# labhamlet/wavjepa

Measured on AMD Instinct MI355X. Metric: jepa_pretrain_clips_per_sec, higher is better.
Workload: dtype bf16; 1 GPU; WavJEPA-base JEPA pre-training step, 2.01 s @16 kHz white-noise clips (32159 samples -> 200 tokens), 256 clips per GPU (32 sources x 8 crops), AudioSet masker, random-init weights; workload_name=2s-bf16, global_batch=256, seq_len=200, parallelism=dp1, persistent_gemm_workgroups_per_xcd=32

## Files before the change

### wavjepa_amd/csrc/conv0.hip

```cpp
#include <string.h>
#include "conv_pieces.h"
#include "../../include/wavjepa_hip.h"

namespace {

constexpr int TC = 256;
constexpr int NTH = 256;

struct Geo {
    int N, C_in, L, C, k, stride, L_out, P;
    long clip_stride;
};

template <int NT, class T>
__device__ __forceinline__ void stage_steps(T* xs, const bf16_t* __restrict__ audio, const Geo& g, int n, int t0, int span) {
    stage_chunk<NT>(xs, audio, (long)n * g.clip_stride, g.C_in, g.L, (long)t0 * g.stride, span);
}

__host__ __device__ constexpr long fwd_record(int C, int taps, int want_yx) { return want_yx ? 2L * C + (long)C * taps + taps : 2L * C; }

constexpr int STATS_SLOTS = 768;
inline int stats_tcs(int N, int L_out, int C_in) {
    static int forced = -1;
    if (forced < 0) forced = wj_lab_env_int("WJ_CONV0_STATS_TCS", 0);
    if (forced >= 32) return forced / 32 * 32;
    int chunks = (STATS_SLOTS + N / 2) / (N > 0 ? N : 1);
    const int most = (L_out + 255) / 256;
    chunks = chunks < 1 ? 1 : (chunks > most ? most : chunks);
    const int tcs = ((L_out + chunks - 1) / chunks + 31) / 32 * 32;
    const int cap = 2176 / (C_in > 0 ? C_in : 1) / 32 * 32;
    return tcs > cap ? (cap < 32 ? 32 : cap) : tcs;
}
inline int stats_chunks(int L_out, int TCS) { return (L_out + TCS - 1) / TCS; }
template <int TAPS>
__global__ __launch_bounds__(256) void conv0_gram_kernel(const bf16_t* __restrict__ audio, double* __restrict__ part, Geo g, int span, int TCS) {
    extern __shared__ __attribute__((aligned(16))) bf16_t xa[];
    constexpr int G = TAPS + TAPS * TAPS;
    __shared__ double red[4][G];
    const int n = blockIdx.y, t0 = blockIdx.x * TCS;
    stage_steps<256>(xa, audio, g, n, t0, span);
    __syncthreads();
    const int lane = threadIdx.x & 63, wave = threadIdx.x >> 6;
    const int tcount = min(TCS, g.L_out - t0);
    for (int p = lane; p < G; p += 64) {
        const bool one = p < TAPS;
        const int qa = one ? p : (p - TAPS) / TAPS, qb = one ? 0 : (p - TAPS) - qa * TAPS;
        const int offa = tap_at(qa, g.k, span), offb = tap_at(qb, g.k, span);
        double acc = 0.0;
        for (int t = wave; t < tcount; t += 4) {
            const float a = bf2f(xa[offa + t * g.stride]);
            const float b = one ? 1.0f : bf2f(xa[offb + t * g.stride]);
            acc += (double)(a * b);
        }
        red[wave][p] = acc;
    }
    __syncthreads();
    double* o = part + ((long)n * gridDim.x + blockIdx.x) * G;
    for (int p = threadIdx.x; p < G; p += 256) o[p] = (red[0][p] + red[1][p]) + (red[2][p] + red[3][p]);
}

template <int TAPS>
__global__ __launch_bounds__(256) void conv0_stats_from_gram_kernel(const double* __restrict__ gram, const bf16_t* __restrict__ wsrc,
                                                                    float* __restrict__ sums, float* __restrict__ yx, float* __restrict__ x1,
                                                                    Geo g) {
    constexpr int G = TAPS + TAPS * TAPS;
    __shared__ double gs[G];
    const int n = blockIdx.y;
    for (int p = threadIdx.x; p < G; p += 256) gs[p] = gram[(long)n * G + p];
    __syncthreads();
    if (x1 && blockIdx.x == 0 && threadIdx.x < TAPS) x1[(long)n * TAPS + threadIdx.x] = (float)gs[threadIdx.x];
    const int c = blockIdx.x * 256 + threadIdx.x;
    if (c >= g.C) return;
    double w[TAPS];
#pragma unroll
    for (int q = 0; q < TAPS; ++q) w[q] = (double)bf2f(wsrc[(long)c * TAPS + q]);
    double s1 = 0.0, s2 = 0.0;
#pragma unroll
    for (int q = 0; q < TAPS; ++q) s1 += w[q] * gs[q];
#pragma unroll
    for (int q = 0; q < TAPS; ++q) {
        double v = 0.0;
#pragma unroll
        for (int k = 0; k < TAPS; ++k) v += w[k] * gs[TAPS + k * TAPS + q];
        s2 += v * w[q];
        if (yx) yx[((long)n * g.C + c) * TAPS + q] = (float)v;
    }
    sums[((long)n * g.C + c) * 2] = (float)s1;
    sums[((long)n * g.C + c) * 2 + 1] = (float)fmax(s2, 0.0);
}

template <int TAPS>
__global__ __launch_bounds__(256) void conv0_stats_mfma_kernel(const bf16_t* __restrict__ audio, const bf16_t* __restrict__ wsrc,
                                                               float* __restrict__ part, int want_yx, Geo g, int span, int TCS) {
    extern __shared__ __attribute__((aligned(16))) bf16_t xa[];
    constexpr int QT = (TAPS + 15) / 16;
    const int n = blockIdx.y, t0 = blockIdx.x * TCS;
    const long rec = fwd_record(g.C, TAPS, want_yx);
    float* sums = part + ((long)n * gridDim.x + blockIdx.x) * rec;
    float* yx = want_yx ? sums + 2L * g.C : nullptr;
    float* x1 = want_yx ? yx + (long)g.C * TAPS : nullptr;
    stage_steps<256>(xa, audio, g, n, t0, span);
    __syncthreads();
    const int lane = threadIdx.x & 63, wave = threadIdx.x >> 6, i = lane & 15, gq = lane >> 4;
    const int tcount = min(TCS, g.L_out - t0);
    const bf16_t zero = f2bf(0.f);
    int offc[8];
    bool okc[8];
    tap_map<TAPS>(offc, okc, 8 * gq, 1, g.k, span);
    int offq[QT];
    bool okq[QT];
    tap_map<TAPS>(offq, okq, i, 16, g.k, span);
    const int ntile = g.C / 16;
    for (int ctg = wave * 8; ctg < ntile; ctg += 32) {
        bf16x8 wf[8];
#pragma unroll
        for (int u = 0; u < 8; ++u)
#pragma unroll
            for (int j = 0; j < 8; ++j)
                wf[u][j] = (ctg + u < ntile && okc[j]) ? wsrc[(long)((ctg + u) * 16 + i) * TAPS + 8 * gq + j] : zero;
        f32x4 yxa[8][QT];
        float s1[8], s2[8], xs1[QT];
#pragma unroll
        for (int u = 0; u < 8; ++u) {
            s1[u] = s2[u] = 0.f;
#pragma unroll
            for (int qt = 0; qt < QT; ++qt) yxa[u][qt] = f32x4{0.f, 0.f, 0.f, 0.f};
        }
#pragma unroll
        for (int qt = 0; qt < QT; ++qt) xs1[qt] = 0.f;
        for (int tb = 0; tb < tcount; tb += 32) {
            bf16x8 p0, p1, pq[QT];
            const bool v0 = tb + i < tcount, v1 = tb + 16 + i < tcount;
#pragma unroll
            for (int j = 0; j < 8; ++j) {
                p0[j] = (v0 && okc[j]) ? xa[offc[j] + (tb + i) * g.stride] : zero;
                p1[j] = (v1 && okc[j]) ? xa[offc[j] + (tb + 16 + i) * g.stride] : zero;
            }
#pragma unroll
            for (int qt = 0; qt < QT; ++qt)
#pragma unroll
                for (int j = 0; j < 8; ++j) {
                    const int tt = tb + (j < 4 ? 4 * gq + j : 12 + 4 * gq + j);
                    pq[qt][j] = (okq[qt] && tt < tcount) ? xa[offq[qt] + tt * g.stride] : zero;
                }
            if (yx && ctg == 0) {
#pragma unroll
                for (int qt = 0; qt < QT; ++qt)
#pragma unroll
                    for (int j = 0; j < 8; ++j) xs1[qt] += bf2f(pq[qt][j]);
            }
#pragma unroll
            for (int u = 0; u < 8; ++u) {
                const f32x4 z4 = f32x4{0.f, 0.f, 0.f, 0.f};
                const f32x4 d0 = __builtin_amdgcn_mfma_f32_16x16x32_bf16(p0, wf[u], z4, 0, 0, 0);
                const f32x4 d1 = __builtin_amdgcn_mfma_f32_16x16x32_bf16(p1, wf[u], z4, 0, 0, 0);
                bf16x8 yq;
#pragma unroll
                for (int r = 0; r < 4; ++r) {
                    yq[r] = f2bf(d0[r]);
                    yq[4 + r] = f2bf(d1[r]);
                    const float a = bf2f(yq[r]), b = bf2f(yq[4 + r]);
                    s1[u] += a + b;
                    s2[u] = fmaf(a, a, fmaf(b, b, s2[u]));
                }
                if (yx) {
#pragma unroll
                    for (int qt = 0; qt < QT; ++qt) yxa[u][qt] = __builtin_amdgcn_mfma_f32_16x16x32_bf16(pq[qt], yq, yxa[u][qt], 0, 0, 0);
                }
            }
        }
#pragma unroll
        for (int u = 0; u < 8; ++u) {
            if (ctg + u >= ntile) continue;
            const int c = (ctg + u) * 16 + i;
            float a = s1[u], b = s2[u];
            a += __shfl_xor(a, 16, 64); a += __shfl_xor(a, 32, 64);
            b += __shfl_xor(b, 16, 64); b += __shfl_xor(b, 32, 64);
            if (gq == 0) {
                sums[c * 2 + 0] = a;
                sums[c * 2 + 1] = b;
            }
            if (yx) {
#pragma unroll
                for (int qt = 0; qt < QT; ++qt)
#pragma unroll
                    for (int r = 0; r < 4; ++r) {
                        const int q = 16 * qt + 4 * gq + r;
                        if (q < TAPS) yx[(long)c * TAPS + q] = yxa[u][qt][r];
                    }
            }
        }
        if (yx && ctg == 0) {
#pragma unroll
            for (int qt = 0; qt < QT; ++qt) {
                float v = xs1[qt];
                v += __shfl_xor(v, 16, 64); v += __shfl_xor(v, 32, 64);
                if (gq == 0 && okq[qt]) x1[16 * qt + i] = v;
            }
        }
    }
}

template <int TAPS>
__global__ __launch_bounds__(NTH) void conv0_apply_kernel(const bf16_t* __restrict__ audio, const bf16_t* __restrict__ wsrc,
                                                          const float* __restrict__ gamma, const float* __restrict__ beta,
                                                          const float* __restrict__ sums, bf16_t* __restrict__ act,
                                                          float* __restrict__ mean_o, float* __restrict__ rstd_o, Geo g,
                                                          int span_max, float eps) {
    extern __shared__ float xs[];
    const int n = blockIdx.y, t0 = blockIdx.x * TC;
    const int half = threadIdx.x >> 7, cl = threadIdx.x & 127;
    stage_steps<NTH>(xs, audio, g, n, t0, span_max);
    __syncthreads();
    const int tmax = min(TC, g.P - t0);
    const float invL = 1.0f / (float)g.L_out;
    for (int cb = 0; cb < g.C; cb += 512) {
        const int c4 = cb + cl * 4;
        if (c4 >= g.C) continue;
        float w[4][TAPS];
        load_weights(w, wsrc, c4);
        float mu[4], rs[4], ga[4], be[4];
// ... 126 lines not shown
    extern __shared__ float xs[];
    int* tl = reinterpret_cast<int*>(xs + BR * TAPS);
    float* red = xs + BR * TAPS + BR;
    const int n = blockIdx.y;
    const int first = rows ? row_off[n] : 0;
    const int cnt = rows ? row_off[n + 1] - first : g.L_out;
    const int j0 = blockIdx.x * BR;
    if (j0 >= cnt) return;
    const int jn = min(BR, cnt - j0);
    const int half = threadIdx.x >> 7, cl = threadIdx.x & 127;
    for (int j = threadIdx.x; j < jn; j += NTH) tl[j] = rows ? rows[first + j0 + j] - n * g.P : j0 + j;
    __syncthreads();
    for (int idx = threadIdx.x; idx < jn * TAPS; idx += NTH) {
        const int j = idx / TAPS;
        xs[idx] = bf2f(audio[(long)n * g.clip_stride + (long)tl[j] * g.stride + tap_at(idx - j * TAPS, g.k, g.L)]);
    }
    __syncthreads();
    for (int cb = 0; cb < g.C; cb += 512) {
        const int c4 = cb + cl * 4;
        const bool live = c4 < g.C;
        float acc[4][TAPS], a1[4] = {0, 0, 0, 0}, a2[4] = {0, 0, 0, 0};
#pragma unroll
        for (int j = 0; j < 4; ++j)
#pragma unroll
            for (int tp = 0; tp < TAPS; ++tp) acc[j][tp] = 0.f;
        if (live) {
            float w[4][TAPS];
            load_weights(w, wsrc, c4);
            float mu[4], rs[4], ga[4], be[4];
#pragma unroll
            for (int j = 0; j < 4; ++j) {
                mu[j] = mean[(long)n * g.C + c4 + j]; rs[j] = rstd[(long)n * g.C + c4 + j];
                ga[j] = gamma[c4 + j]; be[j] = beta[c4 + j];
            }
            constexpr int RB = 4;
            for (int jj0 = half; jj0 < jn; jj0 += 2 * RB) {
                bf16x4 dv[RB];
#pragma unroll
                for (int u = 0; u < RB; ++u) {
                    const int jq = jj0 + 2 * u < jn ? jj0 + 2 * u : jj0;
                    dv[u] = *reinterpret_cast<const bf16x4*>(dact + ((long)n * g.P + tl[jq]) * g.C + c4);
                }
#pragma unroll
                for (int u = 0; u < RB; ++u) {
                    const int jj = jj0 + 2 * u;
                    if (jj >= jn) break;
                    float x[TAPS], y[4];
#pragma unroll
                    for (int tp = 0; tp < TAPS; ++tp) x[tp] = xs[jj * TAPS + tp];
                    conv_row(y, x, [&](int j, int q) { return w[j][q]; }, nullptr);
                    const bf16x4 d = dv[u];
#pragma unroll
                    for (int j = 0; j < 4; ++j) {
                        const float xh = (y[j] - mu[j]) * rs[j];
                        const float dz = bf2f(d[j]) * gelu_grad_f(xh * ga[j] + be[j]);
                        a1[j] += dz;
                        a2[j] = fmaf(dz, xh, a2[j]);
#pragma unroll
                        for (int tp = 0; tp < TAPS; ++tp) acc[j][tp] = fmaf(dz, x[tp], acc[j][tp]);
                    }
                }
            }
        }
        __syncthreads();
        if (live && half == 1) {
#pragma unroll
            for (int j = 0; j < 4; ++j) {
                red[(j * (2 + TAPS) + 0) * 128 + cl] = a1[j];
                red[(j * (2 + TAPS) + 1) * 128 + cl] = a2[j];
#pragma unroll
                for (int tp = 0; tp < TAPS; ++tp) red[(j * (2 + TAPS) + 2 + tp) * 128 + cl] = acc[j][tp];
            }
        }
        __syncthreads();
        if (live && half == 0) {
#pragma unroll
            for (int j = 0; j < 4; ++j) {
                float* o = ws + (((long)n * gridDim.x + blockIdx.x) * g.C + c4 + j) * (2 + TAPS);
                o[0] = a1[j] + red[(j * (2 + TAPS) + 0) * 128 + cl];
                o[1] = a2[j] + red[(j * (2 + TAPS) + 1) * 128 + cl];
#pragma unroll
                for (int tp = 0; tp < TAPS; ++tp) o[2 + tp] = acc[j][tp] + red[(j * (2 + TAPS) + 2 + tp) * 128 + cl];
            }
        }
    }
}

template <int TAPS>
__global__ __launch_bounds__(256) void conv0_bwd_final_kernel(const float* __restrict__ gamma, const float* __restrict__ mean,
                                                              const float* __restrict__ rstd, const float* __restrict__ ws,
                                                              const float* __restrict__ yx, const float* __restrict__ x1,
                                                              float* __restrict__ dw, float* __restrict__ dgamma,
                                                              float* __restrict__ dbeta, Geo g) {
    __shared__ float r0[8][33], r1[8][33], r2[8][33];
    const int pl = threadIdx.x & 31, nl = threadIdx.x >> 5;
    const int pair = blockIdx.x * 32 + pl;
    const int c = pair / TAPS, tp = pair - c * TAPS;
    const bool live = c < g.C;
    const float invL = 1.0f / (float)g.L_out;
    float sw = 0.f, sg = 0.f, sb = 0.f;
    if (live) {
        const float ga = gamma[c];
        for (int n = nl; n < g.N; n += 8) {
            const float* o = ws + ((long)n * g.C + c) * (2 + TAPS);
            const float A1 = o[0], A2 = o[1], S = o[2 + tp];
            const float mu = mean[(long)n * g.C + c], rs = rstd[(long)n * g.C + c];
            const float X1 = x1[(long)n * TAPS + tp], YX = yx[((long)n * g.C + c) * TAPS + tp];
            sw += rs * ga * (S - A1 * invL * X1 - A2 * invL * rs * (YX - mu * X1));
            sg += A2;
            sb += A1;
        }
    }
    r0[nl][pl] = sw; r1[nl][pl] = sg; r2[nl][pl] = sb;
    __syncthreads();
    if (nl == 0 && live) {
        float a = 0.f, b = 0.f, d = 0.f;
#pragma unroll
        for (int i = 0; i < 8; ++i) { a += r0[i][pl]; b += r1[i][pl]; d += r2[i][pl]; }
        dw[(long)c * TAPS + tp] += a;
        if (tp == 0) {
            dgamma[c] += b;
            dbeta[c] += d;
        }
    }
}

template <class A>
Geo geo_of(const A* a) {
    return Geo{a->N, a->C_in, a->L, a->C, a->k, a->stride, a->L_out, a->P, packed_clip_stride(a->audio_clip_stride, a->C_in, a->L)};
}

template <int TAPS, int MINB>
void launch_apply_mfma(const wj_conv0_fwd_args* a, const Geo& g, const float* sums, hipStream_t s) {
    const int span = (TCA - 1) * a->stride + a->k;
    hipLaunchKernelGGL((conv0_apply_mfma_kernel<TAPS, MINB>), dim3((a->P + TCA - 1) / TCA, a->N), dim3(512), (size_t)a->C_in * span * sizeof(bf16_t),
                       s, (const bf16_t*)a->audio, (const bf16_t*)a->w, a->gamma, a->beta, sums, (bf16_t*)a->act, a->mean, a->rstd, g, span, a->eps);
}

template <int TAPS>
void launch_fwd(const wj_conv0_fwd_args* a, const Geo& g, int span_max, hipStream_t s) {
    const size_t lds = (size_t)a->C_in * span_max * sizeof(float);
    dim3 grid2((a->P + TC - 1) / TC, a->N), block(NTH);
    const int want_yx = a->yx != nullptr;
    const int TCS = stats_tcs(a->N, a->L_out, a->C_in);
    const int chunks = stats_chunks(a->L_out, TCS);
    const long rec = fwd_record(a->C, TAPS, want_yx);
    float* sums = a->workspace;
    float* part = a->workspace + 2L * a->N * a->C;
    const int span = (TCS - 1) * a->stride + a->k;
    static const int gram_mode = [] { const char* e = getenv("WJ_CONV0_STATS"); return (e && !strcmp(e, "mfma")) ? 0 : 1; }();
    constexpr long G = TAPS + (long)TAPS * TAPS;
    if (gram_mode && 2 * G * (chunks + 1) <= (long)chunks * fwd_record(a->C, TAPS, 1)) {
        double* gpart = reinterpret_cast<double*>(part);
        double* gfold = gpart + (long)a->N * chunks * G;
        hipLaunchKernelGGL(conv0_gram_kernel<TAPS>, dim3(chunks, a->N), dim3(256), (size_t)a->C_in * span * sizeof(bf16_t), s,
                           (const bf16_t*)a->audio, gpart, g, span, TCS);
        fold_records(s, 1, a->N, (const double*)gpart, chunks, G, gfold, G);
        hipLaunchKernelGGL(conv0_stats_from_gram_kernel<TAPS>, dim3((a->C + 255) / 256, a->N), dim3(256), 0, s, (const double*)gfold,
                           (const bf16_t*)a->w, sums, a->yx, a->x1, g);
    } else {
        hipLaunchKernelGGL(conv0_stats_mfma_kernel<TAPS>, dim3(chunks, a->N), dim3(256), (size_t)a->C_in * span * sizeof(bf16_t), s,
                           (const bf16_t*)a->audio, (const bf16_t*)a->w, part, want_yx, g, span, TCS);
        fold_records(s, (unsigned)((rec + 1023) / 1024), a->N, (const float*)part, chunks, rec, sums, 2L * a->C, a->yx, (long)a->C * TAPS, a->x1);
    }
    static const int use_mfma = wj_lab_env_int("WJ_CONV0_APPLY_MFMA", 1);
    if (use_mfma && a->C % 64 == 0 && TAPS <= 32) {
        static const int occ = wj_lab_env_int("WJ_CONV0_APPLY_OCC", 1);
        if (occ >= 2) launch_apply_mfma<TAPS, 2>(a, g, sums, s);
        else launch_apply_mfma<TAPS, 1>(a, g, sums, s);
        return;
    }
    hipLaunchKernelGGL(conv0_apply_kernel<TAPS>, grid2, block, lds, s, (const bf16_t*)a->audio, (const bf16_t*)a->w,
                       a->gamma, a->beta, (const float*)sums, (bf16_t*)a->act, a->mean, a->rstd, g, span_max, a->eps);
}

constexpr long bwd_record(int C, int taps) { return (long)C * (2 + taps); }
inline int bwd_chunks(int max_rows) { return (max_rows + BR - 1) / BR; }

template <int TAPS>
void launch_bwd(const wj_conv0_bwd_args* a, const Geo& g, hipStream_t s) {
    const size_t lds = (size_t)(BR * TAPS + BR + (2 + TAPS) * 4 * 128) * sizeof(float);
    const int max_rows = a->rows ? a->max_rows : a->L_out;
    if (max_rows <= 0) return;
    static int attr = hipFuncSetAttribute((const void*)conv0_bwd_rows_kernel<TAPS>, hipFuncAttributeMaxDynamicSharedMemorySize, (int)lds);
    (void)attr;
    const int chunks = bwd_chunks(max_rows);
    const long rec = bwd_record(a->C, TAPS);
    float* folded = a->workspace;
    float* part = a->workspace + (long)a->N * rec;
    dim3 grid(chunks, a->N), block(NTH);
    hipLaunchKernelGGL(conv0_bwd_rows_kernel<TAPS>, grid, block, lds, s, (const bf16_t*)a->audio, (const bf16_t*)a->w, a->gamma,
                       a->beta, a->mean, a->rstd, (const bf16_t*)a->dact, a->rows, a->row_off, part, g);
    fold_records(s, (unsigned)((rec + 1023) / 1024), a->N, (const float*)part, chunks, rec, folded, rec, (float*)nullptr, 0L, (float*)nullptr,
                 a->rows ? a->row_off : (const int32_t*)nullptr, BR);
    hipLaunchKernelGGL(conv0_bwd_final_kernel<TAPS>, dim3((a->C * TAPS + 31) / 32), dim3(256), 0, s, a->gamma, a->mean, a->rstd,
                       (const float*)folded, a->yx, a->x1, a->dw, a->dgamma, a->dbeta, g);
}

}

int64_t wj_conv0_fwd_ws_bytes(const wj_conv0_fwd_args* a) {
    if (a->L_out <= 0) return -1;
    const int chunks = stats_chunks(a->L_out, stats_tcs(a->N, a->L_out, a->C_in));
    const long rec = fwd_record(a->C, a->C_in * a->k, 1);
    return (2L * a->N * a->C + (long)a->N * chunks * rec) * 4;
}
int64_t wj_conv0_bwd_ws_bytes(const wj_conv0_bwd_args* a) {
    const int max_rows = a->max_rows > 0 ? a->max_rows : a->L_out;
    return (long)a->N * (1 + bwd_chunks(max_rows)) * bwd_record(a->C, a->C_in * a->k) * 4;
}

extern "C" int wj_conv0_gn_gelu_fwd(const wj_conv0_fwd_args* a, void* stream) {
    WJ_CLEAR_STALE_ERROR();
    if (!a || !a->audio || !a->w || !a->gamma || !a->beta || !a->act || !a->mean || !a->rstd || !a->workspace) return WJ_ERR_ARG;
    if (a->N <= 0 || a->C <= 0 || (a->C & 15) || a->L_out <= 0 || a->P < a->L_out) return WJ_ERR_ARG;
    if ((a->L_out - 1) * a->stride + a->k > a->L) return WJ_ERR_ARG;
    hipStream_t s = (hipStream_t)stream;
    const Geo g = geo_of(a);
    const int span_max = (TC - 1) * a->stride + a->k;
    if ((a->yx == nullptr) != (a->x1 == nullptr)) return WJ_ERR_ARG;
    if (!taps_dispatch(a->C_in * a->k, [&](auto taps) { launch_fwd<decltype(taps)::value>(a, g, span_max, s); })) return WJ_ERR_UNSUPPORTED;
    WJ_CHECK_LAUNCH();
    return WJ_OK;
}

extern "C" int wj_conv0_gn_gelu_bwd(const wj_conv0_bwd_args* a, void* stream) {
    WJ_CLEAR_STALE_ERROR();
    if (!a || !a->audio || !a->w || !a->gamma || !a->beta || !a->mean || !a->rstd || !a->dact || !a->dw || !a->dgamma ||
        !a->dbeta || !a->workspace || !a->yx || !a->x1)
        return WJ_ERR_ARG;
    if (a->N <= 0 || a->C <= 0 || (a->C & 3) || a->L_out <= 0 || a->P < a->L_out) return WJ_ERR_ARG;
    if (a->rows && (!a->row_off || a->max_rows < 0)) return WJ_ERR_ARG;
    hipStream_t s = (hipStream_t)stream;
    const Geo g = geo_of(a);
    if (!taps_dispatch(a->C_in * a->k, [&](auto taps) { launch_bwd<decltype(taps)::value>(a, g, s); })) return WJ_ERR_UNSUPPORTED;
    WJ_CHECK_LAUNCH();
    return WJ_OK;
}
```

### wavjepa_amd/csrc/misc.hip

```cpp
#include "common.h"
#include "../../include/wavjepa_hip.h"
#ifdef WJ_LAB
#include "../../include/wavjepa_hip_lab.h"
#endif

namespace {

inline int grid_for(long n_items, int per_block, int cap = 8192) {
    long g = (n_items + per_block - 1) / per_block;
    if (g < 1) g = 1;
    return (int)(g > cap ? cap : g);
}

__global__ __launch_bounds__(256) void gelu_bwd_kernel(const bf16_t* __restrict__ dpost, const bf16_t* __restrict__ pre,
                                                       bf16_t* __restrict__ dpre, long n8) {
    for (long i = blockIdx.x * 256L + threadIdx.x; i < n8; i += (long)gridDim.x * 256) {
        const bf16x8 d = *reinterpret_cast<const bf16x8*>(dpost + i * 8);
        const bf16x8 p = *reinterpret_cast<const bf16x8*>(pre + i * 8);
        bf16x8 o;
#pragma unroll
        for (int e = 0; e < 8; ++e) o[e] = f2bf(bf2f(d[e]) * gelu_grad_f(bf2f(p[e])));
        *reinterpret_cast<bf16x8*>(dpre + i * 8) = o;
    }
}
// ... 123 lines not shown
                tok = f32x4{bf2f(v[0]), bf2f(v[1]), bf2f(v[2]), bf2f(v[3])};
            } else {
                const f32x4 mt = *reinterpret_cast<const f32x4*>(a.mask_token + c);
                tok = f32x4{bf2f(f2bf(mt[0])), bf2f(f2bf(mt[1])), bf2f(f2bf(mt[2])), bf2f(f2bf(mt[3]))};
            }
            const f32x4 y = tok + *reinterpret_cast<const f32x4*>(a.pos + (long)t * D + c);
            bf16x4 yb;
#pragma unroll
            for (int e = 0; e < 4; ++e) yb[e] = f2bf(y[e]);
            if (a.out_f32) *reinterpret_cast<f32x4*>(a.out_f32 + (long)r * D + c) = y;
            if (a.out_bf16) *reinterpret_cast<bf16x4*>((bf16_t*)a.out_bf16 + (long)r * D + c) = yb;
        }
    }
}

constexpr int SFB_WROWS = 4;
constexpr int SFB_ROWS = 4 * SFB_WROWS;
template <int JMAX>
__global__ __launch_bounds__(256) void scatter_fill_bwd_kernel(wj_scatter_fill_bwd_args a) {
    extern __shared__ float macc_dyn[];
    const int lane = threadIdx.x & 63, wave = __builtin_amdgcn_readfirstlane(threadIdx.x >> 6);
    const int D = a.D, M = a.B * a.T, G = a.G;
    const int m0 = blockIdx.x * SFB_ROWS + wave * SFB_WROWS;
    int idx = -1;
    {
        const int r = lane / (G + 1), u = lane - r * (G + 1), m = m0 + r;
        if (r < SFB_WROWS && m < M) {
            if (u == G) {
                idx = a.inv[m];
            } else {
                const int b = m / a.T, t = m - b * a.T;
                const int row = (b * G + u) * a.T + t;
                idx = a.rowmap ? a.rowmap[row] : row;
            }
        }
    }
    f32x4 mt[JMAX];
#pragma unroll
    for (int j = 0; j < JMAX; ++j) mt[j] = f32x4{0.f, 0.f, 0.f, 0.f};
#pragma unroll
    for (int r = 0; r < SFB_WROWS; ++r) {
        if (m0 + r >= M) break;
        const int dst = __builtin_amdgcn_readlane(idx, r * (G + 1) + G);
        f32x4 s[JMAX];
#pragma unroll
        for (int j = 0; j < JMAX; ++j) s[j] = f32x4{0.f, 0.f, 0.f, 0.f};
        for (int g0 = 0; g0 < G; g0 += 4) {
            f32x4 v[4][JMAX];
            bool ok[4];
#pragma unroll
            for (int u = 0; u < 4; ++u) {
                const int g = g0 + u;
                const int row = g < G ? __builtin_amdgcn_readlane(idx, r * (G + 1) + (g < G ? g : 0)) : -1;
                ok[u] = row >= 0;
                const float* src = a.d_in + (long)(ok[u] ? row : 0) * D;
#pragma unroll
                for (int j = 0; j < JMAX; ++j) {
                    const int c = lane * 4 + 256 * j;
                    v[u][j] = f32x4{0.f, 0.f, 0.f, 0.f};
                    if (c < D) v[u][j] = *reinterpret_cast<const f32x4*>(src + c);
                }
            }
#pragma unroll
            for (int u = 0; u < 4; ++u)
#pragma unroll
                for (int j = 0; j < JMAX; ++j)
                    if (ok[u]) s[j] += v[u][j];
        }
#pragma unroll
        for (int j = 0; j < JMAX; ++j) {
            const int c = lane * 4 + 256 * j;
            if (c < D) {
                if (dst >= 0) {
                    bf16x4 o;
#pragma unroll
                    for (int e = 0; e < 4; ++e) o[e] = f2bf(s[j][e]);
                    *reinterpret_cast<bf16x4*>((bf16_t*)a.d_ctx_feats + (long)dst * D + c) = o;
                } else {
                    mt[j] += s[j];
                }
            }
        }
    }
    if (!a.d_mask_token) return;
#pragma unroll
    for (int j = 0; j < JMAX; ++j) {
        const int c = lane * 4 + 256 * j;
        if (c < D) *reinterpret_cast<f32x4*>(&macc_dyn[wave * D + c]) = mt[j];
    }
    __syncthreads();
    for (int c = threadIdx.x; c < D; c += 256) {
        const float v = (macc_dyn[c] + macc_dyn[D + c]) + (macc_dyn[2 * D + c] + macc_dyn[3 * D + c]);
        if (a.partials) a.partials[(long)blockIdx.x * D + c] = v;
        else atomicAdd(a.d_mask_token + c, v);
    }
}

__global__ __launch_bounds__(256) void unmask_rows_kernel(wj_unmask_rows_args a) {
    const int D4 = a.D / 4;
    const long n = (long)a.M * D4;
    for (long i = blockIdx.x * 256L + threadIdx.x; i < n; i += (long)gridDim.x * 256) {
        const int m = (int)(i / D4), c = (int)(i - (long)m * D4) * 4;
        const int src = a.inv ? a.inv[m] : m;
        f32x4 y = f32x4{0.f, 0.f, 0.f, 0.f};
        if (src >= 0) {
            if (a.src_is_f32) {
                y = *reinterpret_cast<const f32x4*>((const float*)a.src + (long)src * a.D + c);
            } else {
                const bf16x4 v = *reinterpret_cast<const bf16x4*>((const bf16_t*)a.src + (long)src * a.D + c);
                y = f32x4{bf2f(v[0]), bf2f(v[1]), bf2f(v[2]), bf2f(v[3])};
            }
        }
        if (a.dst_is_bf16) {
            bf16x4 o;
#pragma unroll
            for (int e = 0; e < 4; ++e) o[e] = f2bf(y[e]);
            *reinterpret_cast<bf16x4*>((bf16_t*)a.dst + (long)m * a.D + c) = o;
        } else {
            *reinterpret_cast<f32x4*>((float*)a.dst + (long)m * a.D + c) = y;
        }
    }
}

__global__ __launch_bounds__(1024) void instnorm_kernel(wj_instnorm_args a) {
    __shared__ float red[16];
    const long base = (long)blockIdx.x * a.TD;
    const float* x = a.x + base;
    const int n4 = a.TD / 4;
    float s = 0.f;
    for (int i = threadIdx.x; i < n4; i += 1024) {
        const f32x4 v = *reinterpret_cast<const f32x4*>(x + i * 4);
        s += v[0] + v[1] + v[2] + v[3];
    }
    const float mean = block_sum(s, red) / (float)a.TD;
    float q = 0.f;
    for (int i = threadIdx.x; i < n4; i += 1024) {
        const f32x4 v = *reinterpret_cast<const f32x4*>(x + i * 4);
#pragma unroll
        for (int e = 0; e < 4; ++e) { const float d = v[e] - mean; q += d * d; }
    }
    const float var = block_sum(q, red) / (float)a.TD;
    const float k = rsqrtf(var + a.eps) * a.scale;
    float* t = a.targets + base;
    for (int i = threadIdx.x; i < n4; i += 1024) {
        const f32x4 v = *reinterpret_cast<const f32x4*>(x + i * 4);
        f32x4 o;
#pragma unroll
        for (int e = 0; e < 4; ++e) o[e] = (v[e] - mean) * k;
        if (a.accumulate) o += *reinterpret_cast<const f32x4*>(t + i * 4);
        *reinterpret_cast<f32x4*>(t + i * 4) = o;
    }
}

__global__ __launch_bounds__(256) void instnorm_mean_kernel(wj_instnorm_mean_args a) {
    const int b = blockIdx.y;
    const float* xs[8] = {a.x0, a.x1, a.x2, a.x3, a.x4, a.x5, a.x6, a.x7};
    const float invn = 1.0f / (float)a.TD, invk = 1.0f / (float)a.K;
    float mu[8], sc[8];
#pragma unroll
    for (int l = 0; l < 8; ++l) {
        mu[l] = sc[l] = 0.f;
        if (l < a.K) {
            float s1 = 0.f, s2 = 0.f;
#pragma unroll
            for (int p = 0; p < WJ_GROUP_STATS_SPLIT; ++p) {
                s1 += a.stats[(((long)l * a.B + b) * WJ_GROUP_STATS_SPLIT + p) * 2];
                s2 += a.stats[(((long)l * a.B + b) * WJ_GROUP_STATS_SPLIT + p) * 2 + 1];
            }
            mu[l] = s1 * invn;
            sc[l] = rsqrtf(fmaxf(s2 * invn - mu[l] * mu[l], 0.f) + a.eps) * invk;
        }
    }
    const long base = (long)b * a.TD;
    const int n4 = a.TD / 4;
    for (int i = blockIdx.x * 256 + threadIdx.x; i < n4; i += gridDim.x * 256) {
        f32x4 o = f32x4{0.f, 0.f, 0.f, 0.f};
#pragma unroll
        for (int l = 0; l < 8; ++l) {
            if (l < a.K) {
                const f32x4 v = *reinterpret_cast<const f32x4*>(xs[l] + base + i * 4);
#pragma unroll
                for (int e = 0; e < 4; ++e) o[e] = fmaf(v[e] - mu[l], sc[l], o[e]);
            }
        }
        *reinterpret_cast<f32x4*>(a.targets + base + i * 4) = o;
    }
}

__global__ __launch_bounds__(1024) void mse_count_kernel(const uint8_t* __restrict__ tgt, float* __restrict__ ws, long n) {
    __shared__ float red[16];
    int k = 0;
    const bool vec = (reinterpret_cast<uintptr_t>(tgt) & 15) == 0;
    const long nv = vec ? n >> 4 : 0;
    for (long i = threadIdx.x; i < nv; i += 1024) {
        const uint4 v = reinterpret_cast<const uint4*>(tgt)[i];
        const uint32_t w[4] = {v.x, v.y, v.z, v.w};
#pragma unroll
        for (int e = 0; e < 4; ++e) {
            const uint32_t nz = (w[e] | (w[e] >> 1) | (w[e] >> 2) | (w[e] >> 3) | (w[e] >> 4) | (w[e] >> 5) | (w[e] >> 6) | (w[e] >> 7)) & 0x01010101u;
            k += __popc(nz);
        }
    }
    for (long i = (nv << 4) + threadIdx.x; i < n; i += 1024) k += tgt[i] ? 1 : 0;
    float c = block_sum((float)k, red);
    if (threadIdx.x == 0) ws[1] = c;
}

template <int KIND>
__device__ __forceinline__ void loss_elem(float d, float beta, float ib, float& e, float& g) {
    if constexpr (KIND == WJ_LOSS_MSE) {
        e = d * d;
        g = d;
    } else {
        const float ad = fabsf(d);
        const float sg = d > 0.f ? 1.0f : (d < 0.f ? -1.0f : 0.f);
        if constexpr (KIND == WJ_LOSS_L1) {
            e = ad;
            g = sg;
        } else if constexpr (KIND == WJ_LOSS_SMOOTH_L1) {
            const float q = d * ib;
            const bool quad = ad < beta;
            e = quad ? (0.5f * d) * q : ad - 0.5f * beta;
            g = quad ? q : sg;
        } else {
            const bool quad = ad <= beta;
            e = quad ? (0.5f * d) * d : beta * (ad - 0.5f * beta);
            g = quad ? d : beta * sg;
        }
    }
}

template <int KIND>
__global__ __launch_bounds__(256) void loss_rows_kernel(wj_loss_args a) {
    const int lane = threadIdx.x & 63, wave = threadIdx.x >> 6;
    const int D = a.D;
    const long R = a.rows ? (long)a.n_rows : (long)a.B * a.G * a.T;
    const float count = a.workspace[1];
    const float gk = (KIND == WJ_LOSS_MSE ? 2.0f : 1.0f) / ((float)D * (count + 1e-8f)) * a.gscale * (a.gscale_ptr ? a.gscale_ptr[0] : 1.0f);
    const float beta = a.beta, ib = KIND == WJ_LOSS_SMOOTH_L1 ? 1.0f / a.beta : 0.f;
    for (long r = blockIdx.x * 4L + wave; r < R; r += gridDim.x * 4L) {
        const long dense = a.rows ? (long)a.rows[r] : r;
        const int t = (int)(dense % a.T);
        const long bg = dense / a.T;
        const int b = (int)(bg / a.G);
        const bool on = a.tgt[dense] != 0;
        float err = 0.f;
        for (int c = lane * 4; c < D; c += 256) {
            bf16x4 dp;
#pragma unroll
            for (int e = 0; e < 4; ++e) dp[e] = f2bf(0.f);
            if (on) {
                const bf16x4 p = *reinterpret_cast<const bf16x4*>((const bf16_t*)a.preds + r * D + c);
                const f32x4 y = *reinterpret_cast<const f32x4*>(a.targets + ((long)b * a.T + t) * D + c);
#pragma unroll
                for (int e = 0; e < 4; ++e) {
                    const float d = bf2f(p[e]) - y[e];
                    float le, lg;
                    loss_elem<KIND>(d, beta, ib, le, lg);
                    err += le;
                    dp[e] = f2bf(lg * gk);
                }
            }
            if (a.dpreds) *reinterpret_cast<bf16x4*>((bf16_t*)a.dpreds + r * D + c) = dp;
        }
        err = wave_sum(err);
        if (lane == 0) a.workspace[2 + r] = on ? err / (float)D : 0.f;
    }
}

__global__ __launch_bounds__(1024) void mse_final_kernel(float* __restrict__ ws, float* __restrict__ loss, long R) {
    __shared__ float red[16];
    float s = 0.f;
    for (long i = threadIdx.x; i < R; i += 1024) s += ws[2 + i];
    s = block_sum(s, red);
    if (threadIdx.x == 0) {
        loss[0] = s / (ws[1] + 1e-8f);
        loss[1] = ws[1];
    }
}

__global__ __launch_bounds__(256) void ema_kernel(wj_ema_args a) {
    const long n4 = a.n / 4;
    const float r = a.r, q = 1.0f - a.r;
    for (long i = blockIdx.x * 256L + threadIdx.x; i < n4; i += (long)gridDim.x * 256) {
        const f32x4 s = *reinterpret_cast<const f32x4*>(a.student + i * 4);
        f32x4 t = *reinterpret_cast<const f32x4*>(a.teacher + i * 4);
#pragma unroll
        for (int e = 0; e < 4; ++e) t[e] = t[e] * r + q * s[e];
        *reinterpret_cast<f32x4*>(a.teacher + i * 4) = t;
        if (a.teacher_bf16) {
            bf16x4 o;
#pragma unroll
            for (int e = 0; e < 4; ++e) o[e] = f2bf(t[e]);
            *reinterpret_cast<bf16x4*>((bf16_t*)a.teacher_bf16 + i * 4) = o;
        }
    }
}

__global__ __launch_bounds__(256) void sumsq_partial_kernel(const float* __restrict__ g, float* __restrict__ ws, long n) {
    __shared__ float red[16];
    const long n4 = n / 4;
    float s = 0.f;
    for (long i = blockIdx.x * 256L + threadIdx.x; i < n4; i += (long)gridDim.x * 256) {
        const f32x4 v = *reinterpret_cast<const f32x4*>(g + i * 4);
        s += v[0] * v[0] + v[1] * v[1] + v[2] * v[2] + v[3] * v[3];
    }
    s = block_sum(s, red);
    if (threadIdx.x == 0) ws[blockIdx.x] = s;
}
__global__ __launch_bounds__(1024) void sumsq_final_kernel(const float* __restrict__ ws, float* __restrict__ out, int n, int accumulate) {
    __shared__ float red[16];
    float s = 0.f;
    for (int i = threadIdx.x; i < n; i += 1024) s += ws[i];
    s = block_sum(s, red);
    if (threadIdx.x == 0) out[0] = accumulate ? out[0] + s : s;
}

__global__ __launch_bounds__(256) void adamw_kernel(wj_adamw_args a) {
    const long n4 = a.n / 4;
    float coef = a.grad_scale;
    if (a.max_norm > 0.f && a.sumsq) {
        const float norm = sqrtf(a.sumsq[0]) * a.grad_scale;
        coef *= fminf(1.0f, a.max_norm / (norm + 1e-6f));
    }
    const float decay = 1.0f - a.lr * a.weight_decay;
    const float step = a.lr / a.bc1;
    const float rbc2 = rsqrtf(a.bc2);
    for (long i = blockIdx.x * 256L + threadIdx.x; i < n4; i += (long)gridDim.x * 256) {
        f32x4 p = *reinterpret_cast<const f32x4*>(a.p + i * 4);
        const f32x4 g = *reinterpret_cast<const f32x4*>(a.g + i * 4);
        if (a.zero_grad) *reinterpret_cast<f32x4*>(a.g + i * 4) = f32x4{0.f, 0.f, 0.f, 0.f};
        f32x4 m = *reinterpret_cast<const f32x4*>(a.m + i * 4);
        f32x4 v = *reinterpret_cast<const f32x4*>(a.v + i * 4);
#pragma unroll
        for (int e = 0; e < 4; ++e) {
            const float ge = g[e] * coef;
            p[e] *= decay;
// ... 110 lines not shown
    const unsigned long long t0 = __builtin_amdgcn_s_memtime();
    while ((long)(__builtin_amdgcn_s_memtime() - t0) < ticks) __builtin_amdgcn_s_sleep(8);
}

extern "C" int wj_spin(const wj_spin_args* a, void* stream) {
    WJ_CLEAR_STALE_ERROR();
    if (!a || a->ticks < 0 || a->ticks > (1LL << 32)) return WJ_ERR_ARG;
    hipLaunchKernelGGL(spin_kernel, dim3(1), dim3(64), 0, STREAM, (long)a->ticks);
    WJ_CHECK_LAUNCH();
    return WJ_OK;
}

#ifdef WJ_LAB
typedef __attribute__((ext_vector_type(4))) unsigned cf_u32x4;
__global__ __launch_bounds__(512) void collective_footprint_kernel(cf_u32x4* __restrict__ buf, long n16, long min_ticks, int passes) {
    const unsigned long long t0 = __builtin_amdgcn_s_memrealtime();
    const long per = (n16 + gridDim.x - 1) / gridDim.x;
    const long lo = per * blockIdx.x, hi = min(n16, lo + per);
    constexpr long PIECE = 512 * 8;
    const long npieces = ((hi > lo ? hi - lo : 0) + PIECE - 1) / PIECE * passes;
    long done = 0;
    for (int ps = 0; ps < passes; ++ps)
        for (long p0 = lo; p0 < hi; p0 += PIECE) {
            cf_u32x4 v[8];
#pragma unroll
            for (int u = 0; u < 8; ++u) {
                const long i = p0 + u * 512 + threadIdx.x;
                v[u] = cf_u32x4{0u, 0u, 0u, 0u};
                if (i < hi) v[u] = __builtin_nontemporal_load(buf + i);
            }
#pragma unroll
            for (int u = 0; u < 8; ++u) {
                const long i = p0 + u * 512 + threadIdx.x;
                asm volatile("" : "+v"(v[u].x));
                if (i < hi) __builtin_nontemporal_store(v[u], buf + i);
            }
            ++done;
            if (min_ticks > 0) {
                const unsigned long long due = (unsigned long long)(min_ticks * done / npieces);
                while (__builtin_amdgcn_s_memrealtime() - t0 < due) __builtin_amdgcn_s_sleep(16);
            }
        }
}

extern "C" int wj_collective_footprint(const wj_collective_footprint_args* a, void* stream) {
    WJ_CLEAR_STALE_ERROR();
    if (!a || !a->buf || a->bytes <= 0 || (a->bytes & 15) || ((uintptr_t)a->buf & 15) || a->workgroups < 1 || a->workgroups > 256 ||
        a->passes < 1 || a->passes > 8 || a->min_ticks < 0)
        return WJ_ERR_ARG;
    hipLaunchKernelGGL(collective_footprint_kernel, dim3(a->workgroups), dim3(512), 0, STREAM, (cf_u32x4*)a->buf, (long)(a->bytes / 16),
                       (long)a->min_ticks, a->passes);
    WJ_CHECK_LAUNCH();
    return WJ_OK;
}
#endif

extern "C" int wj_zero_rows(const wj_zero_rows_args* a, void* stream) {
    WJ_CLEAR_STALE_ERROR();
    if (!a || !a->buf || !a->rows || a->n_rows < 0 || a->row_bytes <= 0 || (a->row_bytes & 15)) return WJ_ERR_ARG;
    if (a->n_rows == 0) return WJ_OK;
    hipLaunchKernelGGL(zero_rows_kernel, dim3(grid_for((long)a->n_rows * (a->row_bytes / 16), 256)), dim3(256), 0, STREAM,
                       (char*)a->buf, a->rows, a->n_rows, a->row_bytes / 16);
    WJ_CHECK_LAUNCH();
    return WJ_OK;
}

extern "C" int wj_conv_weight_layout(const wj_conv_w_args* a, void* stream) {
    WJ_CLEAR_STALE_ERROR();
    if (!a || !a->src || !a->dst || a->C_out <= 0 || a->C_in <= 0 || a->k <= 0 || a->mode < 0 || a->mode > 2) return WJ_ERR_ARG;
    if (a->mode == 1 && (a->U <= 0 || a->rho < 0 || a->rho + a->stride * (a->U - 1) >= a->k)) return WJ_ERR_ARG;
    const long n = a->mode == 1 ? (long)a->U * a->C_out * a->C_in : (long)a->C_out * a->C_in * a->k;
    hipLaunchKernelGGL(conv_w_kernel, dim3(grid_for(n, 256, 2048)), dim3(256), 0, STREAM, *a);
    WJ_CHECK_LAUNCH();
    return WJ_OK;
}

extern "C" int wj_add_pos(const wj_add_pos_args* a, void* stream) {
    WJ_CLEAR_STALE_ERROR();
    if (!a || !a->x || !a->pos || a->M <= 0 || a->T <= 0 || a->D <= 0 || (a->D & 3)) return WJ_ERR_ARG;
    hipLaunchKernelGGL(add_pos_kernel, dim3(grid_for((long)a->M * a->D / 4, 256)), dim3(256), 0, STREAM, *a);
    WJ_CHECK_LAUNCH();
    return WJ_OK;
}

extern "C" int wj_mask_gather_rows(const wj_gather_args* a, void* stream) {
    WJ_CLEAR_STALE_ERROR();
    if (!a || !a->x || !a->idx || !a->out || a->n_rows < 0 || a->D <= 0) return WJ_ERR_ARG;
    if (a->elem_bytes != 2 && a->elem_bytes != 4) return WJ_ERR_ARG;
    const int row_bytes = a->D * a->elem_bytes;
    if (row_bytes & 15) return WJ_ERR_ARG;
    if (a->n_rows == 0) return WJ_OK;
    hipLaunchKernelGGL(gather_rows_kernel, dim3(grid_for(a->n_rows, 1, 16384)), dim3(256), 0, STREAM, (const char*)a->x, a->idx,
                       (char*)a->out, a->n_rows, row_bytes);
    WJ_CHECK_LAUNCH();
    return WJ_OK;
}

extern "C" int wj_mask_scatter_fill_pos(const wj_scatter_fill_args* a, void* stream) {
    WJ_CLEAR_STALE_ERROR();
    if (!a || !a->ctx_feats || !a->inv || !a->mask_token || !a->pos || a->B <= 0 || a->T <= 0 || a->D <= 0 || (a->D & 3) ||
        a->G <= 0)
        return WJ_ERR_ARG;
    if (a->rows) {
        if (a->n_rows < 0) return WJ_ERR_ARG;
        if (a->n_rows == 0) return WJ_OK;
        hipLaunchKernelGGL(scatter_fill_rows_kernel, dim3(grid_for((long)a->n_rows, 4)), dim3(256), 0, STREAM, *a);
        WJ_CHECK_LAUNCH();
        return WJ_OK;
    }
    hipLaunchKernelGGL(scatter_fill_kernel, dim3(grid_for((long)a->B * a->T, 4)), dim3(256), 0, STREAM, *a);
    WJ_CHECK_LAUNCH();
    return WJ_OK;
}

extern "C" int wj_scatter_fill_bwd_partial_rows(int B, int T) { return (int)(((long)B * T + SFB_ROWS - 1) / SFB_ROWS); }
int64_t wj_scatter_fill_bwd_ws_bytes(const wj_scatter_fill_bwd_args* a) { return (int64_t)wj_scatter_fill_bwd_partial_rows(a->B, a->T) * a->D * 4; }

extern "C" int wj_mask_scatter_fill_pos_bwd(const wj_scatter_fill_bwd_args* a, void* stream) {
    WJ_CLEAR_STALE_ERROR();
    if (!a || !a->d_in || !a->inv || !a->d_ctx_feats || a->B <= 0 || a->T <= 0 || a->D <= 0 || (a->D & 3) || a->D > 1024 ||
        a->G <= 0 || a->G > 15)
        return WJ_ERR_ARG;
    const int grid = wj_scatter_fill_bwd_partial_rows(a->B, a->T);
    if (a->D <= 512) hipLaunchKernelGGL(scatter_fill_bwd_kernel<2>, dim3(grid), dim3(256), (size_t)4 * a->D * sizeof(float), STREAM, *a);
    else hipLaunchKernelGGL(scatter_fill_bwd_kernel<4>, dim3(grid), dim3(256), (size_t)4 * a->D * sizeof(float), STREAM, *a);
    WJ_CHECK_LAUNCH();
    return WJ_OK;
}

extern "C" int wj_unmask_rows_f32(const wj_unmask_rows_args* a, void* stream) {
    WJ_CLEAR_STALE_ERROR();
    if (!a || !a->src || !a->dst || a->M <= 0 || a->D <= 0 || (a->D & 3)) return WJ_ERR_ARG;
    hipLaunchKernelGGL(unmask_rows_kernel, dim3(grid_for((long)a->M * a->D / 4, 256)), dim3(256), 0, STREAM, *a);
    WJ_CHECK_LAUNCH();
    return WJ_OK;
}

extern "C" int wj_instnorm_accumulate(const wj_instnorm_args* a, void* stream) {
    WJ_CLEAR_STALE_ERROR();
    if (!a || !a->x || !a->targets || a->B <= 0 || a->TD <= 0 || (a->TD & 3)) return WJ_ERR_ARG;
    hipLaunchKernelGGL(instnorm_kernel, dim3(a->B), dim3(1024), 0, STREAM, *a);
    WJ_CHECK_LAUNCH();
    return WJ_OK;
}

extern "C" int wj_instnorm_mean(const wj_instnorm_mean_args* a, void* stream) {
    WJ_CLEAR_STALE_ERROR();
    if (!a || !a->stats || !a->targets || a->B <= 0 || a->TD <= 0 || (a->TD & 3) || a->K < 1 || a->K > 8) return WJ_ERR_ARG;
    const float* xs[8] = {a->x0, a->x1, a->x2, a->x3, a->x4, a->x5, a->x6, a->x7};
    for (int l = 0; l < a->K; ++l)
        if (!xs[l]) return WJ_ERR_ARG;
    int gx = (a->TD / 4 + 255) / 256;
    if (gx > 32) gx = 32;
    hipLaunchKernelGGL(instnorm_mean_kernel, dim3(gx, a->B), dim3(256), 0, STREAM, *a);
    WJ_CHECK_LAUNCH();
    return WJ_OK;
}

static int masked_loss_launch(const wj_loss_args* a, void* stream) {
    if (!a->preds || !a->targets || !a->tgt || !a->loss || !a->workspace) return WJ_ERR_ARG;
    if (a->B <= 0 || a->G <= 0 || a->T <= 0 || a->D <= 0 || (a->D & 3)) return WJ_ERR_ARG;
    const long Rd = (long)a->B * a->G * a->T;
    if (a->rows && a->n_rows < 0) return WJ_ERR_ARG;
    if (a->kind < WJ_LOSS_MSE || a->kind > WJ_LOSS_HUBER) return WJ_ERR_UNSUPPORTED;
    if ((a->kind == WJ_LOSS_SMOOTH_L1 || a->kind == WJ_LOSS_HUBER) && !(a->beta > 0.f && a->beta <= 3.402823466e38f)) return WJ_ERR_ARG;
    const long R = a->rows ? (long)a->n_rows : Rd;
    hipLaunchKernelGGL(mse_count_kernel, dim3(1), dim3(1024), 0, STREAM, a->tgt, a->workspace, Rd);
    if (R > 0) {
        const dim3 grid(grid_for(R, 4));
        switch (a->kind) {
            case WJ_LOSS_MSE: hipLaunchKernelGGL(loss_rows_kernel<WJ_LOSS_MSE>, grid, dim3(256), 0, STREAM, *a); break;
            case WJ_LOSS_L1: hipLaunchKernelGGL(loss_rows_kernel<WJ_LOSS_L1>, grid, dim3(256), 0, STREAM, *a); break;
            case WJ_LOSS_SMOOTH_L1: hipLaunchKernelGGL(loss_rows_kernel<WJ_LOSS_SMOOTH_L1>, grid, dim3(256), 0, STREAM, *a); break;
            default: hipLaunchKernelGGL(loss_rows_kernel<WJ_LOSS_HUBER>, grid, dim3(256), 0, STREAM, *a); break;
        }
    }
    hipLaunchKernelGGL(mse_final_kernel, dim3(1), dim3(1024), 0, STREAM, a->workspace, a->loss, R);
    WJ_CHECK_LAUNCH();
    return WJ_OK;
}

static int64_t masked_loss_ws_bytes(int B, int G, int T) { return (2 + (int64_t)B * G * T) * 4; }
int64_t wj_masked_mse_ws_bytes(const wj_mse_args* a) { return masked_loss_ws_bytes(a->B, a->G, a->T); }
int64_t wj_masked_loss_ws_bytes(const wj_loss_args* a) { return masked_loss_ws_bytes(a->B, a->G, a->T); }

extern "C" int wj_masked_mse(const wj_mse_args* a, void* stream) {
    WJ_CLEAR_STALE_ERROR();
    if (!a) return WJ_ERR_ARG;
    const wj_loss_args l = {a->preds, a->targets, a->tgt, a->rows, a->loss, a->dpreds, a->workspace, a->gscale_ptr,
                            a->B, a->G, a->T, a->D, a->n_rows, a->gscale, WJ_LOSS_MSE, 0.f};
    return masked_loss_launch(&l, stream);
}

extern "C" int wj_masked_loss(const wj_loss_args* a, void* stream) {
    WJ_CLEAR_STALE_ERROR();
    if (!a) return WJ_ERR_ARG;
    return masked_loss_launch(a, stream);
}

extern "C" int wj_ema_update(const wj_ema_args* a, void* stream) {
    WJ_CLEAR_STALE_ERROR();
    if (!a || !a->student || !a->teacher || a->n <= 0 || (a->n & 3)) return WJ_ERR_ARG;
    hipLaunchKernelGGL(ema_kernel, dim3(grid_for(a->n / 4, 256)), dim3(256), 0, STREAM, *a);
    WJ_CHECK_LAUNCH();
    return WJ_OK;
}

constexpr int SUMSQ_MAX_GRID = 1024;
int64_t wj_grad_sumsq_ws_bytes(const wj_sumsq_args*) { return SUMSQ_MAX_GRID * 4; }

extern "C" int wj_grad_sumsq(const wj_sumsq_args* a, void* stream) {
    WJ_CLEAR_STALE_ERROR();
    if (!a || !a->g || !a->out || !a->workspace || a->n <= 0 || (a->n & 3)) return WJ_ERR_ARG;
    int grid = grid_for(a->n / 4, 256, SUMSQ_MAX_GRID);
    if (a->workgroups > 0 && a->workgroups < grid) grid = a->workgroups;
    hipLaunchKernelGGL(sumsq_partial_kernel, dim3(grid), dim3(256), 0, STREAM, a->g, a->workspace, (long)a->n);
    hipLaunchKernelGGL(sumsq_final_kernel, dim3(1), dim3(1024), 0, STREAM, (const float*)a->workspace, a->out, grid, a->accumulate);
    WJ_CHECK_LAUNCH();
    return WJ_OK;
}

extern "C" int wj_adamw_step(const wj_adamw_args* a, void* stream) {
    WJ_CLEAR_STALE_ERROR();
    if (!a || !a->p || !a->g || !a->m || !a->v || a->n <= 0 || (a->n & 3)) return WJ_ERR_ARG;
    int grid = grid_for(a->n / 4, 256);
    if (a->workgroups > 0 && a->workgroups < grid) grid = a->workgroups;
    hipLaunchKernelGGL(adamw_kernel, dim3(grid), dim3(256), 0, STREAM, *a);
    WJ_CHECK_LAUNCH();
    return WJ_OK;
}

extern "C" int wj_transpose_bf16(const wj_transpose_args* a, void* stream) {
    WJ_CLEAR_STALE_ERROR();
    if (!a || !a->src || !a->dst || !a->table || a->n_mats <= 0 || a->n_tiles <= 0) return WJ_ERR_ARG;
    if (((uintptr_t)a->src | (uintptr_t)a->dst) & 15) return WJ_ERR_ARG;
    hipLaunchKernelGGL(transpose_tiles_kernel, dim3(a->n_tiles), dim3(256), 0, STREAM, *a);
    WJ_CHECK_LAUNCH();
    return WJ_OK;
}

extern "C" int wj_cast_f32_to_bf16(const wj_cast_args* a, void* stream) {
    WJ_CLEAR_STALE_ERROR();
    if (!a || !a->src || !a->dst || a->n <= 0) return WJ_ERR_ARG;
    hipLaunchKernelGGL(cast_kernel, dim3(grid_for(a->n / 4 + 1, 256)), dim3(256), 0, STREAM, a->src, (bf16_t*)a->dst, (long)a->n);
    WJ_CHECK_LAUNCH();
    return WJ_OK;
}

extern "C" int wj_crop_normalize_bf16(const wj_crop_args* a, void* stream) {
    WJ_CLEAR_STALE_ERROR();
    if (!a || !a->src || !a->starts || !a->out || a->B <= 0 || a->S <= 0 || a->C <= 0 || a->length <= 1 || a->L_full < a->length)
        return WJ_ERR_ARG;
    hipLaunchKernelGGL(crop_kernel, dim3(a->B * a->S), dim3(1024), 0, STREAM, *a);
    WJ_CHECK_LAUNCH();
    return WJ_OK;
}
```

Before: 5712 clips/s.

## Compute conv0 Gram statistics with FP64 MFMA and fold partials in stats kernel

The conv0 Gram kernel now builds the tap Gram matrix and tap sums with FP64 16x16x4 MFMA tiles. Each lane loads one padded tap, and an extra column of ones gives the X1 sums; previously each lane ran a scalar double loop per Gram entry. The separate fold_records launch is removed, and the stats-from-gram kernel now sums the per-chunk partials itself. Separately, instnorm_mean_kernel is templated on K and loads all layer inputs before accumulating. The MFMA path depends on a tap_at overload taking a template argument, which is not visible in the code shown, and the LDS size grows to hold the per-wave accumulator tiles.

Result: no change. 5667 clips/s (-0.8%).

```diff
diff --git a/wavjepa_amd/csrc/conv0.hip b/wavjepa_amd/csrc/conv0.hip
--- a/wavjepa_amd/csrc/conv0.hip
+++ b/wavjepa_amd/csrc/conv0.hip
@@ -32,41 +32,79 @@
     return tcs > cap ? (cap < 32 ? 32 : cap) : tcs;
 }
 inline int stats_chunks(int L_out, int TCS) { return (L_out + TCS - 1) / TCS; }
+typedef __attribute__((ext_vector_type(4))) double f64x4;
+template <int TAPS>
+constexpr size_t gram_lds(int C_in, int span) {
+    const size_t samples = (size_t)C_in * span * sizeof(bf16_t), tiles = (size_t)4 * (TAPS / 16 + 1) * (TAPS / 16 + 1) * 256 * sizeof(double);
+    return samples > tiles ? samples : tiles;
+}
 template <int TAPS>
 __global__ __launch_bounds__(256) void conv0_gram_kernel(const bf16_t* __restrict__ audio, double* __restrict__ part, Geo g, int span, int TCS) {
     extern __shared__ __attribute__((aligned(16))) bf16_t xa[];
     constexpr int G = TAPS + TAPS * TAPS;
-    __shared__ double red[4][G];
+    constexpr int QT = TAPS / 16 + 1;
+    static_assert(TAPS % 16 != 0, "column TAPS of the padded patch row carries the 1 of X1");
     const int n = blockIdx.y, t0 = blockIdx.x * TCS;
     stage_steps<256>(xa, audio, g, n, t0, span);
     __syncthreads();
-    const int lane = threadIdx.x & 63, wave = threadIdx.x >> 6;
+    const int lane = threadIdx.x & 63, wave = threadIdx.x >> 6, i = lane & 15, gq = lane >> 4;
     const int tcount = min(TCS, g.L_out - t0);
-    for (int p = lane; p < G; p += 64) {
-        const bool one = p < TAPS;
-        const int qa = one ? p : (p - TAPS) / TAPS, qb = one ? 0 : (p - TAPS) - qa * TAPS;
-        const int offa = tap_at(qa, g.k, span), offb = tap_at(qb, g.k, span);
-        double acc = 0.0;
-        for (int t = wave; t < tcount; t += 4) {
-            const float a = bf2f(xa[offa + t * g.stride]);
-            const float b = one ? 1.0f : bf2f(xa[offb + t * g.stride]);
-            acc += (double)(a * b);
-        }
-        red[wave][p] = acc;
-    }
+    int off[QT];
+    bool tap[QT], one[QT];
+#pragma unroll
+    for (int qt = 0; qt < QT; ++qt) {
+        off[qt] = tap_at<TAPS>(16 * qt + i, g.k, span, tap[qt]);
+        one[qt] = 16 * qt + i == TAPS;
+    }
+    f64x4 acc[QT][QT];
+#pragma unroll
+    for (int a = 0; a < QT; ++a)
+#pragma unroll
+        for (int b = 0; b < QT; ++b) acc[a][b] = f64x4{0.0, 0.0, 0.0, 0.0};
+    for (int tb = 4 * wave; tb < tcount; tb += 16) {
+        const int t = tb + gq;
+        double x[QT];
+#pragma unroll
+        for (int qt = 0; qt < QT; ++qt) {
+            x[qt] = 0.0;
+            if (t < tcount) x[qt] = tap[qt] ? (double)bf2f(xa[off[qt] + t * g.stride]) : (one[qt] ? 1.0 : 0.0);
+        }
+#pragma unroll
+        for (int a = 0; a < QT; ++a)
+#pragma unroll
+            for (int b = 0; b < QT; ++b) acc[a][b] = __builtin_amdgcn_mfma_f64_16x16x4f64(x[a], x[b], acc[a][b], 0, 0, 0);
+    }
+    __syncthreads();
+    double* red = reinterpret_cast<double*>(xa);
+#pragma unroll
+    for (int a = 0; a < QT; ++a)
+#pragma unroll
+        for (int b = 0; b < QT; ++b)
+#pragma unroll
+            for (int r = 0; r < 4; ++r) red[((wave * QT * QT + a * QT + b) * 4 + r) * 64 + lane] = acc[a][b][r];
     __syncthreads();
     double* o = part + ((long)n * gridDim.x + blockIdx.x) * G;
-    for (int p = threadIdx.x; p < G; p += 256) o[p] = (red[0][p] + red[1][p]) + (red[2][p] + red[3][p]);
-}
-
-template <int TAPS>
-__global__ __launch_bounds__(256) void conv0_stats_from_gram_kernel(const double* __restrict__ gram, const bf16_t* __restrict__ wsrc,
+    for (int idx = threadIdx.x; idx < QT * QT * 256; idx += 256) {
+        const int tile = idx >> 8, r = (idx >> 6) & 3, l = idx & 63;
+        const int qa = 16 * (tile / QT) + 4 * r + (l >> 4), qb = 16 * (tile % QT) + (l & 15);
+        if (qa > TAPS || qb >= TAPS) continue;
+        const double s = (red[idx] + red[QT * QT * 256 + idx]) + (red[2 * QT * QT * 256 + idx] + red[3 * QT * QT * 256 + idx]);
+        o[qa == TAPS ? qb : TAPS + qa * TAPS + qb] = s;
+    }
+}
+
+template <int TAPS>
+__global__ __launch_bounds__(256) void conv0_stats_from_gram_kernel(const double* __restrict__ part, int chunks, const bf16_t* __restrict__ wsrc,
                                                                     float* __restrict__ sums, float* __restrict__ yx, float* __restrict__ x1,
                                                                     Geo g) {
     constexpr int G = TAPS + TAPS * TAPS;
     __shared__ double gs[G];
     const int n = blockIdx.y;
-    for (int p = threadIdx.x; p < G; p += 256) gs[p] = gram[(long)n * G + p];
+    for (int p = threadIdx.x; p < G; p += 256) {
+        double s = 0;
+        for (int ch = 0; ch < chunks; ++ch) s += part[((long)n * chunks + ch) * G + p];
+        gs[p] = s;
+    }
     __syncthreads();
     if (x1 && blockIdx.x == 0 && threadIdx.x < TAPS) x1[(long)n * TAPS + threadIdx.x] = (float)gs[threadIdx.x];
     const int c = blockIdx.x * 256 + threadIdx.x;
@@ -499,11 +537,9 @@
     constexpr long G = TAPS + (long)TAPS * TAPS;
     if (gram_mode && 2 * G * (chunks + 1) <= (long)chunks * fwd_record(a->C, TAPS, 1)) {
         double* gpart = reinterpret_cast<double*>(part);
-        double* gfold = gpart + (long)a->N * chunks * G;
-        hipLaunchKernelGGL(conv0_gram_kernel<TAPS>, dim3(chunks, a->N), dim3(256), (size_t)a->C_in * span * sizeof(bf16_t), s,
+        hipLaunchKernelGGL(conv0_gram_kernel<TAPS>, dim3(chunks, a->N), dim3(256), gram_lds<TAPS>(a->C_in, span), s,
                            (const bf16_t*)a->audio, gpart, g, span, TCS);
-        fold_records(s, 1, a->N, (const double*)gpart, chunks, G, gfold, G);
-        hipLaunchKernelGGL(conv0_stats_from_gram_kernel<TAPS>, dim3((a->C + 255) / 256, a->N), dim3(256), 0, s, (const double*)gfold,
+        hipLaunchKernelGGL(conv0_stats_from_gram_kernel<TAPS>, dim3((a->C + 255) / 256, a->N), dim3(256), 0, s, (const double*)gpart, chunks,
                            (const bf16_t*)a->w, sums, a->yx, a->x1, g);
     } else {
         hipLaunchKernelGGL(conv0_stats_mfma_kernel<TAPS>, dim3(chunks, a->N), dim3(256), (size_t)a->C_in * span * sizeof(bf16_t), s,
diff --git a/wavjepa_amd/csrc/misc.hip b/wavjepa_amd/csrc/misc.hip
--- a/wavjepa_amd/csrc/misc.hip
+++ b/wavjepa_amd/csrc/misc.hip
@@ -299,37 +299,34 @@
     }
 }
 
+template <int K>
 __global__ __launch_bounds__(256) void instnorm_mean_kernel(wj_instnorm_mean_args a) {
     const int b = blockIdx.y;
     const float* xs[8] = {a.x0, a.x1, a.x2, a.x3, a.x4, a.x5, a.x6, a.x7};
-    const float invn = 1.0f / (float)a.TD, invk = 1.0f / (float)a.K;
-    float mu[8], sc[8];
-#pragma unroll
-    for (int l = 0; l < 8; ++l) {
-        mu[l] = sc[l] = 0.f;
-        if (l < a.K) {
-            float s1 = 0.f, s2 = 0.f;
-#pragma unroll
-            for (int p = 0; p < WJ_GROUP_STATS_SPLIT; ++p) {
-                s1 += a.stats[(((long)l * a.B + b) * WJ_GROUP_STATS_SPLIT + p) * 2];
-                s2 += a.stats[(((long)l * a.B + b) * WJ_GROUP_STATS_SPLIT + p) * 2 + 1];
-            }
-            mu[l] = s1 * invn;
-            sc[l] = rsqrtf(fmaxf(s2 * invn - mu[l] * mu[l], 0.f) + a.eps) * invk;
-        }
+    const float invn = 1.0f / (float)a.TD, invk = 1.0f / (float)K;
+    float mu[K], sc[K];
+#pragma unroll
+    for (int l = 0; l < K; ++l) {
+        float s1 = 0.f, s2 = 0.f;
+#pragma unroll
+        for (int p = 0; p < WJ_GROUP_STATS_SPLIT; ++p) {
+            s1 += a.stats[(((long)l * a.B + b) * WJ_GROUP_STATS_SPLIT + p) * 2];
+            s2 += a.stats[(((long)l * a.B + b) * WJ_GROUP_STATS_SPLIT + p) * 2 + 1];
+        }
+        mu[l] = s1 * invn;
+        sc[l] = rsqrtf(fmaxf(fmaf(-mu[l], mu[l], s2 * invn), 0.f) + a.eps) * invk;
     }
     const long base = (long)b * a.TD;
     const int n4 = a.TD / 4;
     for (int i = blockIdx.x * 256 + threadIdx.x; i < n4; i += gridDim.x * 256) {
+        f32x4 v[K];
+#pragma unroll
+        for (int l = 0; l < K; ++l) v[l] = *reinterpret_cast<const f32x4*>(xs[l] + base + i * 4);
         f32x4 o = f32x4{0.f, 0.f, 0.f, 0.f};
 #pragma unroll
-        for (int l = 0; l < 8; ++l) {
-            if (l < a.K) {
-                const f32x4 v = *reinterpret_cast<const f32x4*>(xs[l] + base + i * 4);
-#pragma unroll
-                for (int e = 0; e < 4; ++e) o[e] = fmaf(v[e] - mu[l], sc[l], o[e]);
-            }
-        }
+        for (int l = 0; l < K; ++l)
+#pragma unroll
+            for (int e = 0; e < 4; ++e) o[e] = fmaf(v[l][e] - mu[l], sc[l], o[e]);
         *reinterpret_cast<f32x4*>(a.targets + base + i * 4) = o;
     }
 }
@@ -746,7 +743,17 @@
         if (!xs[l]) return WJ_ERR_ARG;
     int gx = (a->TD / 4 + 255) / 256;
     if (gx > 32) gx = 32;
-    hipLaunchKernelGGL(instnorm_mean_kernel, dim3(gx, a->B), dim3(256), 0, STREAM, *a);
+    const dim3 grid(gx, a->B);
+    switch (a->K) {
+        case 1: hipLaunchKernelGGL(instnorm_mean_kernel<1>, grid, dim3(256), 0, STREAM, *a); break;
+        case 2: hipLaunchKernelGGL(instnorm_mean_kernel<2>, grid, dim3(256), 0, STREAM, *a); break;
+        case 3: hipLaunchKernelGGL(instnorm_mean_kernel<3>, grid, dim3(256), 0, STREAM, *a); break;
+        case 4: hipLaunchKernelGGL(instnorm_mean_kernel<4>, grid, dim3(256), 0, STREAM, *a); break;
+        case 5: hipLaunchKernelGGL(instnorm_mean_kernel<5>, grid, dim3(256), 0, STREAM, *a); break;
+        case 6: hipLaunchKernelGGL(instnorm_mean_kernel<6>, grid, dim3(256), 0, STREAM, *a); break;
+        case 7: hipLaunchKernelGGL(instnorm_mean_kernel<7>, grid, dim3(256), 0, STREAM, *a); break;
+        default: hipLaunchKernelGGL(instnorm_mean_kernel<8>, grid, dim3(256), 0, STREAM, *a); break;
+    }
     WJ_CHECK_LAUNCH();
     return WJ_OK;
 }
```
